# zkHubHQ/distributed-groth16

Hardware: NVIDIA H100
Metric: G1 MSM throughput (BN254 Pippenger, 2^20 pairs per GPU) (higher is better)
Workload: dtype u32x8 Montgomery (256-bit modular integers)

## Files before the change

distributed_groth16_b200/csrc/msm.cu:

```cuda
#include "common.cuh"
#include "glv.cuh"

namespace b200zk {

static const uint32_t KEY_NONE = 0xFFFFFFFFu;

template <class T>
__device__ __forceinline__ T ld16(const T* p) {
    static_assert(sizeof(T) % 16 == 0, "16-byte multiple");
    T r;
    const uint4* s = reinterpret_cast<const uint4*>(p);
    uint4* d = reinterpret_cast<uint4*>(&r);
#pragma unroll
    for (int i = 0; i < (int)(sizeof(T) / 16); ++i) d[i] = s[i];
    return r;
}
template <class T>
__device__ __forceinline__ void st16(T* p, const T& v) {
    static_assert(sizeof(T) % 16 == 0, "16-byte multiple");
    const uint4* s = reinterpret_cast<const uint4*>(&v);
    uint4* d = reinterpret_cast<uint4*>(p);
#pragma unroll
    for (int i = 0; i < (int)(sizeof(T) / 16); ++i) d[i] = s[i];
}
// ... 107 lines not shown
__global__ void __launch_bounds__(SCAN_THREADS) k_scan_sums(uint32_t* sums, uint32_t n) {
    __shared__ uint32_t warp_sums[32];
    __shared__ uint32_t carry_s;
    if (threadIdx.x == 0) carry_s = 0;
    __syncthreads();
    for (uint32_t base = 0; base < n; base += SCAN_THREADS) {
        uint32_t i = base + threadIdx.x;
        uint32_t v = i < n ? sums[i] : 0, total;
        uint32_t ex = block_exclusive_scan(v, &total, warp_sums);
        uint32_t carry = carry_s;
        if (i < n) sums[i] = ex + carry;
        __syncthreads();
        if (threadIdx.x == 0) carry_s = carry + total;
        __syncthreads();
    }
}
__global__ void __launch_bounds__(SCAN_THREADS) k_scan_add(uint32_t* out, const uint32_t* sums, uint32_t n) {
    uint32_t base = blockIdx.x * SCAN_TILE + threadIdx.x * SCAN_ITEMS;
    uint32_t add = sums[blockIdx.x];
#pragma unroll
    for (uint32_t j = 0; j < SCAN_ITEMS; ++j) if (base + j < n) out[base + j] += add;
}

__global__ void k_msm_scatter(const uint32_t* keys, const uint32_t* ranks, const uint32_t* offsets, uint32_t n, size_t t0,
                              size_t total, uint32_t fold, uint32_t* entries) {
    size_t t = (size_t)blockIdx.x * blockDim.x + threadIdx.x;
    if (t >= total) return;
    t += t0;
    uint32_t key = keys[t];
    if (key == KEY_NONE) return;
    uint32_t i = fold ? (uint32_t)t : (uint32_t)(t % n);
    uint32_t g = key & 0x7FFFFFFFu;
    entries[offsets[g] + ranks[t]] = i | (key & 0x80000000u);
}

static const uint32_t TASK_LEN = 128, MAX_TASK_LEN = 1024;
#ifndef B2_ACC_MINBLOCKS
#define B2_ACC_MINBLOCKS 4
#endif
#ifndef B2_ACC_MINBLOCKS_G2
#define B2_ACC_MINBLOCKS_G2 4
#endif

__global__ void k_msm_task_counts(const uint32_t* offsets, uint32_t nbuckets, uint32_t task_len, uint32_t* ntasks) {
    uint32_t g = blockIdx.x * blockDim.x + threadIdx.x;
    if (g > nbuckets) return;
    ntasks[g] = g < nbuckets ? (offsets[g + 1] - offsets[g] + task_len - 1) / task_len : 0;
}

static const uint32_t MERGE_SMALL = 8;
__global__ void k_msm_fill_tasks(const uint32_t* task_off, uint32_t nbuckets, uint32_t* task_bucket, uint32_t* multi_list,
                                 uint32_t list_cap, uint32_t* multi_count) {
    uint32_t g = blockIdx.x * blockDim.x + threadIdx.x;
    if (g >= nbuckets) return;
    uint32_t lo = task_off[g], hi = task_off[g + 1];
    for (uint32_t t = lo; t < hi; ++t) task_bucket[t] = g;
    if (hi - lo > MERGE_SMALL) multi_list[atomicAdd(multi_count, 1u)] = g;
    else if (hi - lo > 1) multi_list[list_cap - 1 - atomicAdd(multi_count + 1, 1u)] = g;
}

__device__ __forceinline__ uint32_t task_length(const uint32_t* offsets, const uint32_t* task_off, uint32_t g, uint32_t t,
                                                uint32_t task_len) {
    uint32_t lo = offsets[g] + (t - task_off[g]) * task_len, end = offsets[g + 1];
    return (lo + task_len < end ? lo + task_len : end) - lo;
}
__global__ void __launch_bounds__(256) k_msm_task_hist(const uint32_t* offsets, const uint32_t* task_off, const uint32_t* task_bucket,
                                uint32_t nbuckets, uint32_t task_len, uint32_t* hist, uint32_t* task_rank) {
    __shared__ uint32_t sh_cnt[MAX_TASK_LEN + 1], sh_base[MAX_TASK_LEN + 1];
    for (uint32_t i = threadIdx.x; i <= task_len; i += blockDim.x) sh_cnt[i] = 0;
    __syncthreads();
    uint32_t t = blockIdx.x * blockDim.x + threadIdx.x;
    bool live = t < task_off[nbuckets];
    uint32_t len = 0, local = 0;
    if (live) {
        len = task_length(offsets, task_off, task_bucket[t], t, task_len);
        local = atomicAdd(sh_cnt + len, 1u);
    }
    __syncthreads();
    for (uint32_t i = threadIdx.x; i <= task_len; i += blockDim.x)
        if (sh_cnt[i]) sh_base[i] = atomicAdd(hist + i, sh_cnt[i]);
    __syncthreads();
    if (live) task_rank[t] = sh_base[len] + local;
}
__global__ void k_msm_task_hist_scan(uint32_t* hist, uint32_t task_len) {
    uint32_t run = 0;
    for (int len = (int)task_len; len >= 0; --len) { uint32_t c = hist[len]; hist[len] = run; run += c; }
}
__global__ void k_msm_task_order(const uint32_t* offsets, const uint32_t* task_off, const uint32_t* task_bucket,
                                 uint32_t nbuckets, uint32_t task_len, const uint32_t* hist, const uint32_t* task_rank,
                                 uint32_t* order) {
    uint32_t t = blockIdx.x * blockDim.x + threadIdx.x;
    if (t >= task_off[nbuckets]) return;
    uint32_t len = task_length(offsets, task_off, task_bucket[t], t, task_len);
    order[hist[len] + task_rank[t]] = t;
}

template <class F, bool RMW>
__global__ void __launch_bounds__(128, sizeof(F) > 32 ? B2_ACC_MINBLOCKS_G2 : B2_ACC_MINBLOCKS) k_msm_accumulate(const affine_t<F>* bases, const uint32_t* entries, const uint32_t* offsets,
                                 const uint32_t* task_off, const uint32_t* task_bucket, const uint32_t* order,
                                 uint32_t nbuckets, uint32_t task_len, uint32_t wave, xyzz_t<F>* buckets, xyzz_t<F>* task_sums) {
    const uint32_t ntask = task_off[nbuckets];
    const uint32_t nblk = (ntask + blockDim.x - 1) / blockDim.x;
    if (blockIdx.x >= nblk) return;
    uint32_t vb = blockIdx.x;
    const uint32_t stride = nblk / wave;
    if (stride > 1) {
        if (vb < wave) vb *= stride;
        else {
            uint32_t j = vb - wave;
            vb = j < wave * (stride - 1) ? (j / (stride - 1)) * stride + j % (stride - 1) + 1 : wave * stride + (j - wave * (stride - 1));
        }
    }
    uint32_t tid = vb * blockDim.x + threadIdx.x;
    if (tid >= ntask) return;
    uint32_t t = order[tid];
    uint32_t g = task_bucket[t];
    uint32_t t0 = task_off[g], nt = task_off[g + 1] - t0;
    uint32_t lo = offsets[g] + (t - t0) * task_len, end = offsets[g + 1];
    uint32_t hi = lo + task_len < end ? lo + task_len : end;
    xyzz_t<F> acc = xyzz_t<F>::identity();
    if (RMW && nt == 1) acc = ld16(buckets + g);
    for (uint32_t k = lo; k < hi; ++k) {
        uint32_t e = entries[k];
        affine_t<F> p = ld16(bases + (e & 0x7FFFFFFFu));
        xyzz_t<F>::madd(acc, p, (e >> 31) != 0);
    }
    if (nt == 1) st16(buckets + g, acc);
    else st16(task_sums + t, acc);
}

template <class F>
__device__ __forceinline__ xyzz_t<F> add_sel(const xyzz_t<F>& a, const xyzz_t<F>& b) {
    if (sizeof(F) == 32) return xyzz_t<F>::add_inl(a, b);
    return xyzz_t<F>::add(a, b);
}

template <class F>
__global__ void __launch_bounds__(128) k_msm_merge_tasks(const uint32_t* multi_list, const uint32_t* multi_count,
                                  const uint32_t* task_off, const xyzz_t<F>* task_sums, uint32_t rmw, xyzz_t<F>* buckets) {
    __shared__ xyzz_t<F> sh[128];
    uint32_t cnt = *multi_count;
    for (uint32_t i = blockIdx.x; i < cnt; i += gridDim.x) {
        uint32_t g = multi_list[i];
        uint32_t lo = task_off[g], hi = task_off[g + 1];
        xyzz_t<F> acc = xyzz_t<F>::identity();
        for (uint32_t t = lo + threadIdx.x; t < hi; t += 128) acc = add_sel<F>(acc, ld16(task_sums + t));
        sh[threadIdx.x] = acc;
        __syncthreads();
        for (int s = 64; s > 0; s >>= 1) {
            if ((int)threadIdx.x < s) {
                xyzz_t<F> a = sh[threadIdx.x], b = sh[threadIdx.x + s];
                sh[threadIdx.x] = add_sel<F>(a, b);
            }
            __syncthreads();
        }
        if (threadIdx.x == 0) st16(buckets + g, rmw ? add_sel<F>(ld16(buckets + g), sh[0]) : sh[0]);
        __syncthreads();
    }
}

template <class F>
__global__ void __launch_bounds__(128) k_msm_merge_small(const uint32_t* multi_list, uint32_t list_cap, const uint32_t* small_count,
                                                         const uint32_t* task_off, const xyzz_t<F>* task_sums, uint32_t rmw, xyzz_t<F>* buckets) {
    uint32_t cnt = *small_count;
    for (uint32_t i = blockIdx.x * blockDim.x + threadIdx.x; i < cnt; i += gridDim.x * blockDim.x) {
        uint32_t g = multi_list[list_cap - 1 - i];
        uint32_t lo = task_off[g], hi = task_off[g + 1];
        xyzz_t<F> acc = ld16(task_sums + lo);
        for (uint32_t t = lo + 1; t < hi; ++t) acc = add_sel<F>(acc, ld16(task_sums + t));
        if (rmw) acc = add_sel<F>(ld16(buckets + g), acc);
        st16(buckets + g, acc);
    }
}

template <class F>
__global__ void __launch_bounds__(128) k_msm_reduce_segments(const xyzz_t<F>* buckets, uint32_t W, uint32_t B, uint32_t seg_len,
                                      xyzz_t<F>* partials) {
    uint32_t nseg = B / seg_len;
    uint32_t t = blockIdx.x * blockDim.x + threadIdx.x;
    if (t >= W * nseg) return;
    uint32_t w = t / nseg, seg = t % nseg;
    uint32_t lo = seg * seg_len;
    const xyzz_t<F>* bw = buckets + (size_t)w * B;
    xyzz_t<F> run = xyzz_t<F>::identity(), acc = xyzz_t<F>::identity();
    constexpr bool INL = sizeof(F) == 32;
    for (uint32_t k = lo + seg_len; k-- > lo;) {
        xyzz_t<F> bk = ld16(bw + k);
        if (INL) { run = xyzz_t<F>::add_inl(run, bk); acc = xyzz_t<F>::add_inl(acc, run); }
        else { run = xyzz_t<F>::add(run, bk); acc = xyzz_t<F>::add(acc, run); }
    }
    if (lo) {
        xyzz_t<F> m = xyzz_t<F>::identity();
        for (int bit = 31 - __clz(lo); bit >= 0; --bit) {
            if (INL) m = xyzz_t<F>::dbl_inl(m); else m = xyzz_t<F>::dbl(m);
            if ((lo >> bit) & 1) { if (INL) m = xyzz_t<F>::add_inl(m, run); else m = xyzz_t<F>::add(m, run); }
        }
        if (INL) acc = xyzz_t<F>::add_inl(acc, m); else acc = xyzz_t<F>::add(acc, m);
    }
    st16(partials + t, acc);
}

template <class F>
__global__ void __launch_bounds__(128) k_msm_reduce_segments_quad(const xyzz_t<F>* buckets, uint32_t W, uint32_t B, uint32_t seg_len,
                                                                  xyzz_t<F>* partials) {
    typedef quad_ops<F, false> Q;
    __shared__ typename Q::xch_t xch[32];
    typename Q::xch_t* x = &xch[threadIdx.x >> 2];
    const uint32_t nseg = B / seg_len;
    const uint32_t t = (blockIdx.x * blockDim.x + threadIdx.x) >> 2;
    if (t >= W * nseg) return;
    const uint32_t w = t / nseg, seg = t % nseg;
    const uint32_t lo = seg * seg_len;
    const xyzz_t<F>* bw = buckets + (size_t)w * B;
    xyzz_t<F> run = xyzz_t<F>::identity(), acc = xyzz_t<F>::identity();
    for (uint32_t k = lo + seg_len; k-- > lo;) {
        run = Q::add(x, run, ld16(bw + k));
        acc = Q::add(x, acc, run);
    }
    if (lo) {
        xyzz_t<F> m = xyzz_t<F>::identity();
        for (int bit = 31 - __clz(lo); bit >= 0; --bit) {
            m = Q::dbl(x, m);
            if ((lo >> bit) & 1) m = Q::add(x, m, run);
        }
        acc = Q::add(x, acc, m);
    }
    if ((threadIdx.x & 3) == 0) st16(partials + t, acc);
}

template <class F, int THREADS>
__global__ void __launch_bounds__(THREADS) k_msm_window_sum(const xyzz_t<F>* partials, uint32_t nseg, xyzz_t<F>* wsum) {
    __shared__ xyzz_t<F> sh[THREADS];
    const xyzz_t<F>* p = partials + (size_t)blockIdx.x * nseg;
    xyzz_t<F> acc = xyzz_t<F>::identity();
    for (uint32_t i = threadIdx.x; i < nseg; i += THREADS) acc = add_sel<F>(acc, ld16(p + i));
    sh[threadIdx.x] = acc;
    __syncthreads();
    for (int s = THREADS / 2; s > 0; s >>= 1) {
        if ((int)threadIdx.x < s) {
            xyzz_t<F> a = sh[threadIdx.x], b = sh[threadIdx.x + s];
            sh[threadIdx.x] = add_sel<F>(a, b);
        }
        __syncthreads();
    }
    if (threadIdx.x == 0) st16(wsum + blockIdx.x, sh[0]);
}

template <class F>
__global__ void __launch_bounds__(32) k_msm_horner(const xyzz_t<F>* wsum, uint32_t nset, uint32_t c, uint32_t first, uint32_t last,
                                                   xyzz_t<F>* state, xyzz_t<F>* out) {
    typedef quad_ops<F, false> Q;
    __shared__ typename Q::xch_t xch;
    if (blockIdx.x != 0 || threadIdx.x >= 4) return;
    xyzz_t<F> total;
    uint32_t k = 0;
    if (first) { total = ld16(wsum); k = 1; }
    else total = ld16(state);
    for (; k < nset; ++k) {
        for (uint32_t j = 0; j < c; ++j) total = Q::dbl(&xch, total);
        total = Q::add(&xch, total, ld16(wsum + k));
    }
    if (threadIdx.x == 0) st16(last ? out : state, total);
}

__device__ __forceinline__ void glv_phi_x(Fq& x) {
    Fq beta;
#pragma unroll
    for (int i = 0; i < 8; ++i) beta.l[i] = GlvParams::beta(i);
    x = Fq::mul(x, beta);
}
__device__ __forceinline__ void glv_phi_x(Fq2& x) {
    Fq beta;
#pragma unroll
    for (int i = 0; i < 8; ++i) beta.l[i] = GlvParams::beta_g2(i);
    x.c0 = Fq::mul(x.c0, beta);
    x.c1 = Fq::mul(x.c1, beta);
}
template <class F>
__global__ void __launch_bounds__(32) k_msm_horner_glv(const xyzz_t<F>* wsum, uint32_t nwin, uint32_t c, uint32_t first, uint32_t last,
                                                       xyzz_t<F>* state, xyzz_t<F>* out) {
    typedef quad_ops<F, false> Q;
    __shared__ typename Q::xch_t xch[2];
    __shared__ xyzz_t<F> h1;
    if (blockIdx.x != 0 || threadIdx.x >= 8) return;
    const uint32_t half = threadIdx.x >> 2;
    xyzz_t<F> total;
    uint32_t k = 0;
    if (first) { total = ld16(wsum + half); k = 1; }
    else total = ld16(state + half);
    for (; k < nwin; ++k) {
        for (uint32_t j = 0; j < c; ++j) total = Q::dbl(&xch[half], total);
        total = Q::add(&xch[half], total, ld16(wsum + 2 * k + half));
    }
    if (!last) {
        if ((threadIdx.x & 3) == 0) st16(state + half, total);
        return;
    }
    if (threadIdx.x == 4) h1 = total;
    __syncwarp(0xFFu);
    if (half == 0) {
        xyzz_t<F> p = h1;
        if (!p.is_inf()) glv_phi_x(p.x);
        total = Q::add(&xch[0], total, p);
        if (threadIdx.x == 0) st16(out, total);
    }
}

template <class F>
__global__ void k_sum_to_affine(const xyzz_t<F>* pts, uint32_t count, affine_t<F>* out, uint64_t* flag) {
    if (threadIdx.x != 0 || blockIdx.x != 0) return;
    xyzz_t<F> acc = xyzz_t<F>::identity();
    for (uint32_t i = 0; i < count; ++i) acc = xyzz_t<F>::add(acc, ld16(pts + i));
    affine_t<F> a = xyzz_t<F>::to_affine(acc);
    st16(out, a);
    *flag = acc.is_inf() ? 1 : 0;
}

template <class F>
__global__ void k_set_identity(xyzz_t<F>* out) {
    if (threadIdx.x == 0 && blockIdx.x == 0) st16(out, xyzz_t<F>::identity());
}

static unsigned choose_window(size_t n) {
    unsigned lg = ceil_log2(n < 2 ? 2 : n);
    int c = (int)lg - 4;
    if (c < 5) c = 5;
    if (c > 20) c = 20;
    const char* env = getenv("B200ZK_MSM_WINDOW");
    if (env) { int v = atoi(env); if (v >= 2 && v <= 24) c = v; }
    return (unsigned)c;
}

static int exclusive_scan(b200zk_ctx* ctx, cudaStream_t st, const uint32_t* in, uint32_t* out, uint32_t* sums, uint32_t n) {
    uint32_t nblk = (n + SCAN_TILE - 1) / SCAN_TILE;
    {
        LaunchScope ls(ctx, st, "msm_scan");
        k_scan_local<<<nblk, SCAN_THREADS, 0, st>>>(in, out, sums, n);
    }
    {
        LaunchScope ls(ctx, st, "msm_scan");
        k_scan_sums<<<1, SCAN_THREADS, 0, st>>>(sums, nblk);
    }
    {
        LaunchScope ls(ctx, st, "msm_scan");
        k_scan_add<<<nblk, SCAN_THREADS, 0, st>>>(out, sums, n);
    }
    return check_launch(ctx, "scan");
}

static cudaEvent_t msm_event(b200zk_ctx* ctx, int ch, size_t idx) {
    std::vector<cudaEvent_t>& v = ctx->msm_events[ch];
    while (v.size() <= idx) {
        cudaEvent_t e = nullptr;
        if (cudaEventCreateWithFlags(&e, cudaEventDisableTiming) != cudaSuccess) return nullptr;
        v.push_back(e);
    }
    return v[idx];
}

struct MsmStreams {
    cudaStream_t seq, acc;
    bool result_on_seq;
    int channel;
};

struct MsmPart {
    const void* bases;
    const void* scalars;
    size_t n;
    cudaEvent_t bases_ready, scalars_ready;
};

template <class F>
static int msm_dev_impl(b200zk_ctx* ctx, const MsmStreams& ms, DevBuf& ws_buf, const MsmPart* parts, unsigned nparts,
                        void* d_out, const char* acc_name, unsigned tab_c = 0, unsigned c_force = 0) {
    const int ch = ms.channel;
    size_t nev = 0;
    auto next_event = [&]() { return msm_event(ctx, ch, nev++); };
    size_t n = 0, n_max = 0;
    for (unsigned p = 0; p < nparts; ++p) { n += parts[p].n; n_max = parts[p].n > n_max ? parts[p].n : n_max; }
    xyzz_t<F>* out = reinterpret_cast<xyzz_t<F>*>(d_out);
    if (n == 0) {
        cudaStream_t rs = ms.result_on_seq ? ms.seq : ms.acc;
        {
            LaunchScope ls(ctx, rs, "msm_small");
            k_set_identity<F><<<1, 32, 0, rs>>>(out);
        }
        return check_launch(ctx, "k_set_identity");
    }
    if (n >= (1ull << 31)) return set_error(ctx, B200ZK_ERR_ARG, "MSM length must be < 2^31");
    const bool fold = tab_c != 0;
    if (fold && nparts != 1) return set_error(ctx, B200ZK_ERR_ARG, "fixed-base tables take one input part");
    const unsigned c = fold ? tab_c : (c_force ? c_force : choose_window(n));
    static const bool glv_env = !(getenv("B200ZK_MSM_GLV") && getenv("B200ZK_MSM_GLV")[0] == '0');
    static const bool glv2_env = !(getenv("B200ZK_MSM_GLV_G2") && getenv("B200ZK_MSM_GLV_G2")[0] == '0');
    const bool glv = !fold && glv_env && (sizeof(F) == 32 || glv2_env);
    const unsigned Wh = (128 + c - 1) / c;
    const unsigned W = glv ? 2 * Wh : (255 + c - 1) / c;
    const unsigned WB = fold ? 1 : W;
    if ((uint64_t)W * n >= (fold ? (1ull << 31) : (1ull << 32)))
        return set_error(ctx, B200ZK_ERR_ARG, "MSM too large for 32-bit bucket offsets / entry indices (W * n)");
    const uint32_t B = 1u << (c - 1);
    const uint32_t nb = WB * B;
    uint32_t seg_len = B < 16 ? B : 16;
    static const bool quad_env = !(getenv("B200ZK_MSM_QUAD_REDUCE") && getenv("B200ZK_MSM_QUAD_REDUCE")[0] == '0');
    const bool quad_reduce = quad_env && (uint64_t)WB * (B / seg_len) <= 8192;
    {
        static const int seg_env = getenv("B200ZK_MSM_SEG") ? atoi(getenv("B200ZK_MSM_SEG")) : 0;
        if (seg_env >= 2 && (seg_env & (seg_env - 1)) == 0 && (uint32_t)seg_env <= B) seg_len = (uint32_t)seg_env;
        else if (quad_reduce) seg_len = B < 8 ? B : 8;
        else if (ctx->msm_seg_hint && ctx->msm_seg_hint <= B) seg_len = ctx->msm_seg_hint;
    }
    const uint32_t nseg = B / seg_len;
    const uint32_t wsplit = fold ? (nseg >= 16 * 256 ? 16 : (nseg >= 1024 ? 4 : 1)) : 1;

    unsigned ngroups = 1;
    if (!fold && nparts == 1) {
        static const int g_env = getenv("B200ZK_MSM_GROUPS") ? atoi(getenv("B200ZK_MSM_GROUPS")) : 0;
        const unsigned nunits = glv ? Wh : W;
        unsigned want = g_env > 0 ? (unsigned)g_env : (n >= (1u << 22) ? 4u : 1u);
        if (want > nunits) want = nunits;
        ngroups = want;
    }
    const unsigned unit_sets = glv ? 2 : 1;
    const unsigned units = (fold ? 1 : (glv ? Wh : W));
    unsigned bounds[17] = {0};
    bool custom_units = false;
    if (!fold && nparts == 1) {
        static const char* gu_env = getenv("B200ZK_MSM_GROUP_UNITS");
        if (gu_env) {
            unsigned k = 0, sum = 0;
            const char* w = gu_env;
            while (*w && k < 16) {
                unsigned v = (unsigned)strtoul(w, const_cast<char**>(&w), 10);
                if (v) { sum += v; bounds[++k] = sum; }
                while (*w == ',' || *w == ' ') ++w;
            }
            if (k >= 1 && sum == units) { custom_units = true; ngroups = k; }
        }
    }
    auto group_first_unit = [&](unsigned g) {
        return custom_units ? bounds[g] : (unsigned)(((uint64_t)units * g) / ngroups);
    };
    const uint32_t rmw = nparts > 1 ? 1u : 0u;

    const bool split_streams = ms.result_on_seq || ngroups > 1 || nparts > 1;
    const cudaStream_t st = split_streams ? ms.seq : ms.acc, ast = ms.acc;
    const bool handshake = split_streams && !ms.result_on_seq;
    if (handshake) {
        cudaEvent_t e = next_event();
        if (!e) return set_error(ctx, B200ZK_ERR_CUDA, "cudaEventCreate failed");
        B2_CUDA_OK(ctx, cudaEventRecord(e, ast));
        B2_CUDA_OK(ctx, cudaStreamWaitEvent(st, e, 0));
    }
    auto finish = [&]() -> int {
        if (handshake) {
            cudaEvent_t e = next_event();
            if (!e) return set_error(ctx, B200ZK_ERR_CUDA, "cudaEventCreate failed");
            B2_CUDA_OK(ctx, cudaEventRecord(e, st));
            B2_CUDA_OK(ctx, cudaStreamWaitEvent(ast, e, 0));
        }
        return B200ZK_OK;
    };

    auto al = [](size_t x) { return (x + 255) & ~(size_t)255; };
    const size_t total_max = (size_t)W * n_max;
    uint32_t task_len = TASK_LEN;
    while (task_len < MAX_TASK_LEN && (uint64_t)task_len * nb < 3 * (uint64_t)total_max &&
           total_max / (2 * task_len) + nb >= (1u << 19))
        task_len *= 2;
    static const bool short_env = !(getenv("B200ZK_MSM_SHORT_TASKS") && getenv("B200ZK_MSM_SHORT_TASKS")[0] == '0');
    if (short_env && n_max <= (1u << 16))
        while (task_len > 16 && total_max / task_len < (1u << 17)) task_len /= 2;
    const size_t max_tasks = total_max / task_len + nb + ngroups;
    size_t o = 0;
    auto carve = [&](size_t bytes) { size_t r = o; o += al(bytes); return r; };
    struct PartWs { size_t keys, ranks, entries, counts, offsets, ntasks, taskoff, taskbucket, multi, hist, rank, order, tasksums; };
    std::vector<PartWs> pw(nparts);
    for (unsigned p = 0; p < nparts; ++p) {
        const size_t total = (size_t)W * parts[p].n;
        pw[p].keys = carve(total * 4); pw[p].ranks = carve(total * 4); pw[p].entries = carve(total * 4);
        pw[p].counts = carve(((size_t)nb + 1) * 4); pw[p].offsets = carve(((size_t)nb + 1) * 4);
        pw[p].ntasks = carve(((size_t)nb + ngroups) * 4); pw[p].taskoff = carve(((size_t)nb + ngroups) * 4);
        pw[p].taskbucket = carve(max_tasks * 4);
        pw[p].multi = carve((total_max / task_len + 4 * ngroups + 4) * 4);
        pw[p].hist = carve((size_t)ngroups * (MAX_TASK_LEN + 1) * 4);
        pw[p].rank = carve(max_tasks * 4); pw[p].order = carve(max_tasks * 4);
        pw[p].tasksums = carve(max_tasks * sizeof(xyzz_t<F>));
    }
    const size_t o_sums = carve(((size_t)nb / SCAN_TILE + 2) * 4);
    const size_t o_buckets = carve((size_t)nb * sizeof(xyzz_t<F>));
    const size_t o_partials = carve((size_t)WB * nseg * sizeof(xyzz_t<F>));
    const size_t o_wsum = carve((size_t)WB * wsplit * sizeof(xyzz_t<F>));
    const size_t o_state = carve(2 * sizeof(xyzz_t<F>));
    B2_CUDA_OK(ctx, ws_buf.reserve(o));
    char* ws = reinterpret_cast<char*>(ws_buf.p);
    uint32_t* sums = reinterpret_cast<uint32_t*>(ws + o_sums);
    xyzz_t<F>* buckets = reinterpret_cast<xyzz_t<F>*>(ws + o_buckets);
    xyzz_t<F>* partials = reinterpret_cast<xyzz_t<F>*>(ws + o_partials);
    xyzz_t<F>* wsum = reinterpret_cast<xyzz_t<F>*>(ws + o_wsum);
    xyzz_t<F>* hstate = reinterpret_cast<xyzz_t<F>*>(ws + o_state);
    B2_CUDA_OK(ctx, cudaMemsetAsync(buckets, 0, (size_t)nb * sizeof(xyzz_t<F>), st));
    cudaEvent_t buckets_clear = nullptr;
    if (rmw) {
        buckets_clear = next_event();
        if (!buckets_clear) return set_error(ctx, B200ZK_ERR_CUDA, "cudaEventCreate failed");
        B2_CUDA_OK(ctx, cudaEventRecord(buckets_clear, st));
        B2_CUDA_OK(ctx, cudaStreamWaitEvent(ast, buckets_clear, 0));
    }

    struct Group {
        uint32_t set0, nsets, b0, nbk;
        size_t task_cap, task_base;
        uint32_t list_cap; size_t list_base;
    };
    std::vector<Group> groups(ngroups);
    {
        size_t tb = 0, lb = 2 * (size_t)ngroups;
        for (unsigned g = 0; g < ngroups; ++g) {
            Group& G = groups[g];
            const unsigned u0 = group_first_unit(g), u1 = group_first_unit(g + 1);
            G.set0 = u0 * unit_sets; G.nsets = (u1 - u0) * unit_sets;
            G.b0 = G.set0 * B; G.nbk = G.nsets * B;
            const size_t gtotal = fold ? total_max : (size_t)G.nsets * n_max;
            G.task_cap = gtotal / task_len + G.nbk + 1;
            G.task_base = tb; tb += G.task_cap;
            G.list_cap = (uint32_t)(gtotal / task_len + 1);
            G.list_base = lb; lb += G.list_cap;
        }
    }
    std::vector<cudaEvent_t> prepped((size_t)nparts * ngroups), accumulated((size_t)nparts * ngroups);
    for (auto& e : prepped) if (!(e = next_event())) return set_error(ctx, B200ZK_ERR_CUDA, "cudaEventCreate failed");
    for (auto& e : accumulated) if (!(e = next_event())) return set_error(ctx, B200ZK_ERR_CUDA, "cudaEventCreate failed");

    bool l2_window = false;
    if (nparts == 1 && ctx->l2_persist_max && ctx->l2_window_max) {
        size_t bytes = n * sizeof(affine_t<F>);
        cudaStreamAttrValue attr;
        memset(&attr, 0, sizeof(attr));
        attr.accessPolicyWindow.base_ptr = const_cast<void*>(parts[0].bases);
        attr.accessPolicyWindow.num_bytes = bytes < ctx->l2_window_max ? bytes : ctx->l2_window_max;
        double ratio = (double)ctx->l2_persist_max / (double)attr.accessPolicyWindow.num_bytes;
        attr.accessPolicyWindow.hitRatio = ratio > 1.0 ? 1.0f : (float)ratio;
        attr.accessPolicyWindow.hitProp = cudaAccessPropertyPersisting;
        attr.accessPolicyWindow.missProp = cudaAccessPropertyStreaming;
        l2_window = cudaStreamSetAttribute(ast, cudaStreamAttributeAccessPolicyWindow, &attr) == cudaSuccess;
        cudaGetLastError();
    }

    for (unsigned p = 0; p < nparts; ++p) {
        const MsmPart& P = parts[p];
        const size_t np = P.n, total = (size_t)W * np;
        uint32_t* keys = reinterpret_cast<uint32_t*>(ws + pw[p].keys);
        uint32_t* ranks = reinterpret_cast<uint32_t*>(ws + pw[p].ranks);
        uint32_t* entries = reinterpret_cast<uint32_t*>(ws + pw[p].entries);
        uint32_t* counts = reinterpret_cast<uint32_t*>(ws + pw[p].counts);
        uint32_t* offsets = reinterpret_cast<uint32_t*>(ws + pw[p].offsets);
        uint32_t* ntasks_all = reinterpret_cast<uint32_t*>(ws + pw[p].ntasks);
        uint32_t* task_off_all = reinterpret_cast<uint32_t*>(ws + pw[p].taskoff);
        uint32_t* task_bucket_all = reinterpret_cast<uint32_t*>(ws + pw[p].taskbucket);
        uint32_t* multi_all = reinterpret_cast<uint32_t*>(ws + pw[p].multi);
        uint32_t* hist_all = reinterpret_cast<uint32_t*>(ws + pw[p].hist);
        uint32_t* task_rank_all = reinterpret_cast<uint32_t*>(ws + pw[p].rank);
        uint32_t* order_all = reinterpret_cast<uint32_t*>(ws + pw[p].order);
        xyzz_t<F>* task_sums_all = reinterpret_cast<xyzz_t<F>*>(ws + pw[p].tasksums);
        if (np == 0) {
            for (unsigned g = 0; g < ngroups; ++g) {
                B2_CUDA_OK(ctx, cudaEventRecord(prepped[(size_t)p * ngroups + g], st));
                B2_CUDA_OK(ctx, cudaEventRecord(accumulated[(size_t)p * ngroups + g], ast));
            }
            continue;
        }
        if (P.scalars_ready) B2_CUDA_OK(ctx, cudaStreamWaitEvent(st, P.scalars_ready, 0));
        B2_CUDA_OK(ctx, cudaMemsetAsync(counts, 0, ((size_t)nb + 1) * 4, st));
        {
            LaunchScope ls(ctx, st, "msm_digits");
            if (glv) k_msm_digits_glv<<<(unsigned)((np + 255) / 256), 256, 0, st>>>(reinterpret_cast<const Fr*>(P.scalars), (uint32_t)np, c,
                                                                                   Wh, keys, ranks, counts);
            else k_msm_digits<<<(unsigned)((np + 255) / 256), 256, 0, st>>>(reinterpret_cast<const Fr*>(P.scalars), (uint32_t)np, c, W,
                                                                              fold ? 1u : 0u, keys, ranks, counts);
        }
        B2_TRY(check_launch(ctx, "k_msm_digits"));
        B2_TRY(exclusive_scan(ctx, st, counts, offsets, sums, nb + 1));
        B2_CUDA_OK(ctx, cudaMemsetAsync(multi_all, 0, (size_t)ngroups * 8, st));
        B2_CUDA_OK(ctx, cudaMemsetAsync(hist_all, 0, (size_t)ngroups * (MAX_TASK_LEN + 1) * 4, st));

        for (unsigned g = 0; g < ngroups; ++g) {
            const Group& G = groups[g];
            uint32_t* ntasks = ntasks_all + G.b0 + g;
            uint32_t* task_off = task_off_all + G.b0 + g;
            uint32_t* task_bucket = task_bucket_all + G.task_base;
            uint32_t* task_rank = task_rank_all + G.task_base;
            uint32_t* order = order_all + G.task_base;
            uint32_t* hist = hist_all + (size_t)g * (MAX_TASK_LEN + 1);
            {
                LaunchScope ls(ctx, st, "msm_tasks");
                k_msm_task_counts<<<(G.nbk + 1 + 255) / 256, 256, 0, st>>>(offsets + G.b0, G.nbk, task_len, ntasks);
            }
            B2_TRY(check_launch(ctx, "k_msm_task_counts"));
            B2_TRY(exclusive_scan(ctx, st, ntasks, task_off, sums, G.nbk + 1));
            {
                LaunchScope ls(ctx, st, "msm_tasks");
                k_msm_fill_tasks<<<(G.nbk + 255) / 256, 256, 0, st>>>(task_off, G.nbk, task_bucket, multi_all + G.list_base, G.list_cap,
                                                                      multi_all + 2 * g);
            }
            B2_TRY(check_launch(ctx, "k_msm_fill_tasks"));
            {
                LaunchScope ls(ctx, st, "msm_tasks");
                k_msm_task_hist<<<(unsigned)((G.task_cap + 255) / 256), 256, 0, st>>>(offsets + G.b0, task_off, task_bucket, G.nbk, task_len, hist, task_rank);
            }
            {
                LaunchScope ls(ctx, st, "msm_tasks");
                k_msm_task_hist_scan<<<1, 1, 0, st>>>(hist, task_len);
            }
            {
                LaunchScope ls(ctx, st, "msm_tasks");
                k_msm_task_order<<<(unsigned)((G.task_cap + 255) / 256), 256, 0, st>>>(offsets + G.b0, task_off, task_bucket, G.nbk, task_len, hist, task_rank, order);
            }
            B2_TRY(check_launch(ctx, "k_msm_task_order"));
            {
                const size_t t0 = fold ? 0 : (size_t)G.set0 * np, cnt = fold ? total : (size_t)G.nsets * np;
                LaunchScope ls(ctx, st, "msm_scatter");
                k_msm_scatter<<<(unsigned)((cnt + 255) / 256), 256, 0, st>>>(keys, ranks, offsets, (uint32_t)np, t0, cnt, fold ? 1u : 0u, entries);
            }
            B2_TRY(check_launch(ctx, "k_msm_scatter"));
            B2_CUDA_OK(ctx, cudaEventRecord(prepped[(size_t)p * ngroups + g], st));
        }

        if (P.bases_ready) B2_CUDA_OK(ctx, cudaStreamWaitEvent(ast, P.bases_ready, 0));
        for (unsigned g = 0; g < ngroups; ++g) {
            const Group& G = groups[g];
            B2_CUDA_OK(ctx, cudaStreamWaitEvent(ast, prepped[(size_t)p * ngroups + g], 0));
            {
                LaunchScope ls(ctx, ast, acc_name);
                const unsigned grid = (unsigned)((G.task_cap + 127) / 128);
                const uint32_t wave = (uint32_t)ctx->sm_count * (sizeof(F) > 32 ? B2_ACC_MINBLOCKS_G2 : B2_ACC_MINBLOCKS);
                const affine_t<F>* bp = reinterpret_cast<const affine_t<F>*>(P.bases);
                if (rmw) k_msm_accumulate<F, true><<<grid, 128, 0, ast>>>(bp, entries, offsets + G.b0, task_off_all + G.b0 + g, task_bucket_all + G.task_base,
                                                                       order_all + G.task_base, G.nbk, task_len, wave, buckets + G.b0, task_sums_all + G.task_base);
                else k_msm_accumulate<F, false><<<grid, 128, 0, ast>>>(bp, entries, offsets + G.b0, task_off_all + G.b0 + g, task_bucket_all + G.task_base,
                                                                        order_all + G.task_base, G.nbk, task_len, wave, buckets + G.b0, task_sums_all + G.task_base);
            }
            B2_TRY(check_launch(ctx, "k_msm_accumulate"));
            if (rmw) {
                {
                    LaunchScope ls(ctx, ast, "msm_merge");
                    k_msm_merge_tasks<F><<<2 * ctx->sm_count, 128, 0, ast>>>(multi_all + G.list_base, multi_all + 2 * g, task_off_all + G.b0 + g,
                                                                            task_sums_all + G.task_base, rmw, buckets + G.b0);
                }
                {
                    LaunchScope ls(ctx, ast, "msm_merge");
                    k_msm_merge_small<F><<<4 * ctx->sm_count, 128, 0, ast>>>(multi_all + G.list_base, G.list_cap, multi_all + 2 * g + 1,
                                                                            task_off_all + G.b0 + g, task_sums_all + G.task_base, rmw, buckets + G.b0);
                }
                B2_TRY(check_launch(ctx, "k_msm_merge_tasks"));
            }
            B2_CUDA_OK(ctx, cudaEventRecord(accumulated[(size_t)p * ngroups + g], ast));
        }
    }
    if (l2_window) {
        cudaStreamAttrValue attr;
        memset(&attr, 0, sizeof(attr));
        attr.accessPolicyWindow.num_bytes = 0;
        cudaStreamSetAttribute(ast, cudaStreamAttributeAccessPolicyWindow, &attr);
        cudaGetLastError();
    }

    for (unsigned g = 0; g < ngroups; ++g) {
        const Group& G = groups[g];
        for (unsigned p = 0; p < nparts; ++p) B2_CUDA_OK(ctx, cudaStreamWaitEvent(st, accumulated[(size_t)p * ngroups + g], 0));
        if (!rmw) {
            uint32_t* multi_all = reinterpret_cast<uint32_t*>(ws + pw[0].multi);
            uint32_t* task_off = reinterpret_cast<uint32_t*>(ws + pw[0].taskoff) + G.b0 + g;
            xyzz_t<F>* task_sums = reinterpret_cast<xyzz_t<F>*>(ws + pw[0].tasksums) + G.task_base;
            {
                LaunchScope ls(ctx, st, "msm_merge");
                k_msm_merge_tasks<F><<<2 * ctx->sm_count, 128, 0, st>>>(multi_all + G.list_base, multi_all + 2 * g, task_off, task_sums, 0u, buckets + G.b0);
            }
            {
                LaunchScope ls(ctx, st, "msm_merge");
                k_msm_merge_small<F><<<4 * ctx->sm_count, 128, 0, st>>>(multi_all + G.list_base, G.list_cap, multi_all + 2 * g + 1, task_off, task_sums,
                                                                       0u, buckets + G.b0);
            }
            B2_TRY(check_launch(ctx, "k_msm_merge_tasks"));
        }
        {
            LaunchScope ls(ctx, st, "msm_reduce");
            if (quad_reduce)
                k_msm_reduce_segments_quad<F><<<(G.nsets * nseg * 4 + 127) / 128, 128, 0, st>>>(buckets + G.b0, G.nsets, B, seg_len,
                                                                                               partials + (size_t)G.set0 * nseg);
            else
                k_msm_reduce_segments<F><<<(G.nsets * nseg + 127) / 128, 128, 0, st>>>(buckets + G.b0, G.nsets, B, seg_len,
                                                                                      partials + (size_t)G.set0 * nseg);
        }
        B2_TRY(check_launch(ctx, "k_msm_reduce_segments"));
        {
            LaunchScope ls(ctx, st, "msm_window_sum");
            constexpr int T = sizeof(F) > 32 ? 128 : 256;
            k_msm_window_sum<F, T><<<G.nsets * wsplit, T, 0, st>>>(partials + (size_t)G.set0 * nseg, nseg / wsplit, wsum + (size_t)G.set0 * wsplit);
        }
        B2_TRY(check_launch(ctx, "k_msm_window_sum"));
        {
            LaunchScope ls(ctx, st, "msm_combine");
            const uint32_t first = g == 0, last = g + 1 == ngroups;
            if (glv) k_msm_horner_glv<F><<<1, 32, 0, st>>>(wsum + G.set0, G.nsets / 2, c, first, last, hstate, out);
            else k_msm_horner<F><<<1, 32, 0, st>>>(wsum + (size_t)G.set0 * wsplit, G.nsets * wsplit, fold ? 0u : c, first, last, hstate, out);
        }
        B2_TRY(check_launch(ctx, "k_msm_horner"));
    }
    return finish();
}

template <class F>
static int msm_dev_impl(b200zk_ctx* ctx, const MsmStreams& ms, DevBuf& ws_buf, const void* d_bases, const void* d_scalars, size_t n,
                        void* d_out, const char* acc_name, cudaEvent_t bases_ready, cudaEvent_t scalars_ready = nullptr,
                        unsigned tab_c = 0, unsigned c_force = 0) {
    const MsmPart part{d_bases, d_scalars, n, bases_ready, scalars_ready};
    return msm_dev_impl<F>(ctx, ms, ws_buf, &part, 1, d_out, acc_name, tab_c, c_force);
}

static MsmStreams slot_streams(b200zk_ctx* ctx, Slot& sl, int aux) {
    const int ch = 2 * (int)(&sl - ctx->slots) + (aux ? 1 : 0);
    return MsmStreams{ctx->msm_side[ch], aux ? sl.aux_stream : sl.stream, false, ch};
}

int msm_g1_dev(b200zk_ctx* ctx, Slot& sl, const void* d_bases, const void* d_scalars, size_t n, void* d_out,
               cudaEvent_t bases_ready, int aux) {
    return msm_dev_impl<Fq>(ctx, slot_streams(ctx, sl, aux), aux ? sl.ws_msm_aux : sl.ws_msm, d_bases, d_scalars, n, d_out,
                            "msm_accumulate_g1", bases_ready);
}
int msm_g2_dev(b200zk_ctx* ctx, Slot& sl, const void* d_bases, const void* d_scalars, size_t n, void* d_out,
               cudaEvent_t bases_ready, int aux) {
    return msm_dev_impl<Fq2>(ctx, slot_streams(ctx, sl, aux), aux ? sl.ws_msm_aux : sl.ws_msm, d_bases, d_scalars, n, d_out,
                             "msm_accumulate_g2", bases_ready);
}

unsigned msm_table_windows(unsigned c) { return (255 + c - 1) / c; }
unsigned msm_table_auto_window(size_t n) {
    int L = (int)ceil_log2(n < 2 ? 2 : n);
    L = L < 10 ? 10 : (L > 20 ? 20 : L);
    const int cand[4] = {L, L - 1, L + 1, L - 2};
    for (int c : cand) {
        if (c < 10 || c > 20) continue;
        int top = 254 - ((int)msm_table_windows((unsigned)c) - 1) * c;
        if (top >= 6) return (unsigned)c;
    }
    return (unsigned)L;
}

template <class F>
__global__ void __launch_bounds__(128) k_msm_table_build(const affine_t<F>* bases, uint32_t n, uint32_t c, uint32_t W,
                                                         affine_t<F>* table) {
    uint32_t i = blockIdx.x * blockDim.x + threadIdx.x;
    if (i >= n) return;
    affine_t<F> p = ld16(bases + i);
    st16(table + i, p);
    for (uint32_t w = 1; w < W; ++w) {
        if (!p.is_inf()) {
            xyzz_t<F> acc = xyzz_t<F>::from_affine(p);
            for (uint32_t k = 0; k < c; ++k) acc = xyzz_t<F>::dbl(acc);
            p = xyzz_t<F>::to_affine(acc);
        }
        st16(table + (size_t)w * n + i, p);
    }
}

template <class F>
static int table_build_impl(b200zk_ctx* ctx, cudaStream_t st, const void* d_bases, size_t n, unsigned c, void* d_table) {
    if (c < 2 || c > 24) return set_error(ctx, B200ZK_ERR_ARG, "table window must be in [2, 24]");
    if (n == 0) return B200ZK_OK;
    const unsigned W = msm_table_windows(c);
    if ((uint64_t)W * n >= (1ull << 31)) return set_error(ctx, B200ZK_ERR_ARG, "table too large (W * n >= 2^31)");
    {
        LaunchScope ls(ctx, st, "msm_table_build");
        k_msm_table_build<F><<<(unsigned)((n + 127) / 128), 128, 0, st>>>(reinterpret_cast<const affine_t<F>*>(d_bases), (uint32_t)n,
                                                                      c, W, reinterpret_cast<affine_t<F>*>(d_table));
    }
    return check_launch(ctx, "k_msm_table_build");
}
int msm_table_build_dev(b200zk_ctx* ctx, Slot& sl, int g2, const void* d_bases, size_t n, unsigned c, void* d_table) {
    return g2 ? table_build_impl<Fq2>(ctx, sl.stream, d_bases, n, c, d_table)
              : table_build_impl<Fq>(ctx, sl.stream, d_bases, n, c, d_table);
}
int msm_table_dev(b200zk_ctx* ctx, Slot& sl, int g2, const void* d_table, const void* d_scalars, size_t n, unsigned c,
                  void* d_out, int aux) {
    if (c < 2 || c > 24) return set_error(ctx, B200ZK_ERR_ARG, "table window must be in [2, 24]");
    const MsmStreams st = slot_streams(ctx, sl, aux);
    DevBuf& ws = aux ? sl.ws_msm_aux : sl.ws_msm;
    return g2 ? msm_dev_impl<Fq2>(ctx, st, ws, d_table, d_scalars, n, d_out, "msm_accumulate_g2", nullptr, nullptr, c)
              : msm_dev_impl<Fq>(ctx, st, ws, d_table, d_scalars, n, d_out, "msm_accumulate_g1", nullptr, nullptr, c);
}
// ... 206 lines not shown
```

Before: 223.4.

## Replace per-segment offset multiply with hierarchical tree reduction of bucket segments

The segment reduction no longer computes the lo*run correction by double-and-add per thread. It emits both the running sum and the weighted sum for each segment, and a new multi-level shared-memory tree kernel combines segments, applying the offset weights with a few doublings per level. This removes a long serial double-and-add chain per segment and the separate window-sum kernel, at the cost of extra launches per level and larger shared-memory use. The single-threaded task-length histogram scan is also replaced by a block-wide parallel scan.

```diff
diff --git a/distributed_groth16_b200/csrc/msm.cu b/distributed_groth16_b200/csrc/msm.cu
--- a/distributed_groth16_b200/csrc/msm.cu
+++ b/distributed_groth16_b200/csrc/msm.cu
@@ -213,9 +213,24 @@
     __syncthreads();
     if (live) task_rank[t] = sh_base[len] + local;
 }
-__global__ void k_msm_task_hist_scan(uint32_t* hist, uint32_t task_len) {
-    uint32_t run = 0;
-    for (int len = (int)task_len; len >= 0; --len) { uint32_t c = hist[len]; hist[len] = run; run += c; }
+__global__ void __launch_bounds__(SCAN_THREADS) k_msm_task_hist_scan(uint32_t* hist, uint32_t task_len) {
+    constexpr uint32_t ITEMS = (MAX_TASK_LEN + SCAN_THREADS) / SCAN_THREADS;
+    __shared__ uint32_t warp_sums[32];
+    uint32_t v[ITEMS], t = 0;
+#pragma unroll
+    for (uint32_t j = 0; j < ITEMS; ++j) {
+        const uint32_t r = threadIdx.x * ITEMS + j;
+        v[j] = r <= task_len ? hist[task_len - r] : 0;
+        t += v[j];
+    }
+    uint32_t total;
+    uint32_t ex = block_exclusive_scan(t, &total, warp_sums);
+#pragma unroll
+    for (uint32_t j = 0; j < ITEMS; ++j) {
+        const uint32_t r = threadIdx.x * ITEMS + j;
+        if (r <= task_len) hist[task_len - r] = ex;
+        ex += v[j];
+    }
 }
 __global__ void k_msm_task_order(const uint32_t* offsets, const uint32_t* task_off, const uint32_t* task_bucket,
                                  uint32_t nbuckets, uint32_t task_len, const uint32_t* hist, const uint32_t* task_rank,
@@ -306,7 +321,7 @@
 
 template <class F>
 __global__ void __launch_bounds__(128) k_msm_reduce_segments(const xyzz_t<F>* buckets, uint32_t W, uint32_t B, uint32_t seg_len,
-                                      xyzz_t<F>* partials) {
+                                      xyzz_t<F>* ys, xyzz_t<F>* gs) {
     uint32_t nseg = B / seg_len;
     uint32_t t = blockIdx.x * blockDim.x + threadIdx.x;
     if (t >= W * nseg) return;
@@ -320,20 +335,13 @@
         if (INL) { run = xyzz_t<F>::add_inl(run, bk); acc = xyzz_t<F>::add_inl(acc, run); }
         else { run = xyzz_t<F>::add(run, bk); acc = xyzz_t<F>::add(acc, run); }
     }
-    if (lo) {
-        xyzz_t<F> m = xyzz_t<F>::identity();
-        for (int bit = 31 - __clz(lo); bit >= 0; --bit) {
-            if (INL) m = xyzz_t<F>::dbl_inl(m); else m = xyzz_t<F>::dbl(m);
-            if ((lo >> bit) & 1) { if (INL) m = xyzz_t<F>::add_inl(m, run); else m = xyzz_t<F>::add(m, run); }
-        }
-        if (INL) acc = xyzz_t<F>::add_inl(acc, m); else acc = xyzz_t<F>::add(acc, m);
-    }
-    st16(partials + t, acc);
+    st16(ys + t, run);
+    st16(gs + t, acc);
 }
 
 template <class F>
 __global__ void __launch_bounds__(128) k_msm_reduce_segments_quad(const xyzz_t<F>* buckets, uint32_t W, uint32_t B, uint32_t seg_len,
-                                                                  xyzz_t<F>* partials) {
+                                                                  xyzz_t<F>* ys, xyzz_t<F>* gs) {
     typedef quad_ops<F, false> Q;
     __shared__ typename Q::xch_t xch[32];
     typename Q::xch_t* x = &xch[threadIdx.x >> 2];
@@ -356,26 +364,54 @@
         }
         acc = Q::add(x, acc, m);
     }
-    if ((threadIdx.x & 3) == 0) st16(partials + t, acc);
-}
-
-template <class F, int THREADS>
-__global__ void __launch_bounds__(THREADS) k_msm_window_sum(const xyzz_t<F>* partials, uint32_t nseg, xyzz_t<F>* wsum) {
-    __shared__ xyzz_t<F> sh[THREADS];
-    const xyzz_t<F>* p = partials + (size_t)blockIdx.x * nseg;
+    if ((threadIdx.x & 3) == 0) { st16(ys + t, xyzz_t<F>::identity()); st16(gs + t, acc); }
+}
+
+template <class F>
+__global__ void k_msm_reduce_level(const xyzz_t<F>* yin, const xyzz_t<F>* gin, uint32_t lgT, uint32_t lgf, xyzz_t<F>* yout,
+                                   xyzz_t<F>* hout) {
+    typedef quad_ops<F, false> Q;
+    extern __shared__ uint4 smem_raw[];
+    xyzz_t<F>* sY = reinterpret_cast<xyzz_t<F>*>(smem_raw);
+    const uint32_t T = 1u << lgT, tid = threadIdx.x;
+    xyzz_t<F>* sG = sY + T;
+    xyzz_t<F>* sP = sG + T;
+    __shared__ typename Q::xch_t xch;
+    const size_t base = (size_t)blockIdx.x * T;
+    if (tid < T) { sY[tid] = ld16(yin + base + tid); sG[tid] = ld16(gin + base + tid); }
+    __syncthreads();
+    for (uint32_t l = 0; l < lgT; ++l) {
+        const uint32_t nn = T >> (l + 1), jobs = nn * (l + 2);
+        xyzz_t<F> r;
+        uint32_t j = 0, kind = 0;
+        if (tid < jobs) {
+            j = tid % nn; kind = tid / nn;
+            const xyzz_t<F>* src = kind == 0 ? sY : kind == 1 ? sG : sP + T - (T >> (kind - 2));
+            r = add_sel<F>(src[2 * j], src[2 * j + 1]);
+            if (kind == 0) sP[T - (T >> l) + j] = src[2 * j + 1];
+        }
+        __syncthreads();
+        if (tid < jobs) {
+            xyzz_t<F>* dst = kind == 0 ? sY : kind == 1 ? sG : sP + T - (T >> (kind - 2));
+            dst[j] = r;
+        }
+        __syncthreads();
+    }
+    if (tid >= 4) return;
     xyzz_t<F> acc = xyzz_t<F>::identity();
-    for (uint32_t i = threadIdx.x; i < nseg; i += THREADS) acc = add_sel<F>(acc, ld16(p + i));
-    sh[threadIdx.x] = acc;
-    __syncthreads();
-    for (int s = THREADS / 2; s > 0; s >>= 1) {
-        if ((int)threadIdx.x < s) {
-            xyzz_t<F> a = sh[threadIdx.x], b = sh[threadIdx.x + s];
-            sh[threadIdx.x] = add_sel<F>(a, b);
-        }
-        __syncthreads();
-    }
-    if (threadIdx.x == 0) st16(wsum + blockIdx.x, sh[0]);
-}
+    for (int jj = (int)lgT - 1; jj >= 0; --jj) {
+        acc = Q::dbl(&xch, acc);
+        acc = Q::add(&xch, acc, sP[T - (T >> jj)]);
+    }
+    for (uint32_t k = 0; k < lgf; ++k) acc = Q::dbl(&xch, acc);
+    acc = Q::add(&xch, sG[0], acc);
+    if (tid == 0) {
+        st16(hout + blockIdx.x, acc);
+        if (yout) st16(yout + blockIdx.x, sY[0]);
+    }
+}
+template <class F> constexpr uint32_t reduce_level_lgtmax() { return sizeof(F) > 32 ? 7 : 8; }
+template <class F> constexpr size_t reduce_level_smem(uint32_t lgT) { return (size_t)(3u << lgT) * sizeof(xyzz_t<F>); }
 
 template <class F>
 __global__ void __launch_bounds__(32) k_msm_horner(const xyzz_t<F>* wsum, uint32_t nset, uint32_t c, uint32_t first, uint32_t last,
@@ -543,7 +579,8 @@
         else if (ctx->msm_seg_hint && ctx->msm_seg_hint <= B) seg_len = ctx->msm_seg_hint;
     }
     const uint32_t nseg = B / seg_len;
-    const uint32_t wsplit = fold ? (nseg >= 16 * 256 ? 16 : (nseg >= 1024 ? 4 : 1)) : 1;
+    constexpr uint32_t LGT_MAX = reduce_level_lgtmax<F>();
+    const uint32_t nlev2 = nseg > (1u << LGT_MAX) ? nseg >> LGT_MAX : 1;
 
     unsigned ngroups = 1;
     if (!fold && nparts == 1) {
@@ -621,14 +658,16 @@
     }
     const size_t o_sums = carve(((size_t)nb / SCAN_TILE + 2) * 4);
     const size_t o_buckets = carve((size_t)nb * sizeof(xyzz_t<F>));
-    const size_t o_partials = carve((size_t)WB * nseg * sizeof(xyzz_t<F>));
-    const size_t o_wsum = carve((size_t)WB * wsplit * sizeof(xyzz_t<F>));
+    const size_t o_lev1 = carve(2 * (size_t)WB * nseg * sizeof(xyzz_t<F>));
+    const size_t o_lev2 = carve(2 * (size_t)WB * nlev2 * sizeof(xyzz_t<F>));
+    const size_t o_wsum = carve((size_t)WB * sizeof(xyzz_t<F>));
     const size_t o_state = carve(2 * sizeof(xyzz_t<F>));
     B2_CUDA_OK(ctx, ws_buf.reserve(o));
     char* ws = reinterpret_cast<char*>(ws_buf.p);
     uint32_t* sums = reinterpret_cast<uint32_t*>(ws + o_sums);
     xyzz_t<F>* buckets = reinterpret_cast<xyzz_t<F>*>(ws + o_buckets);
-    xyzz_t<F>* partials = reinterpret_cast<xyzz_t<F>*>(ws + o_partials);
+    xyzz_t<F>* lev1 = reinterpret_cast<xyzz_t<F>*>(ws + o_lev1);
+    xyzz_t<F>* lev2 = reinterpret_cast<xyzz_t<F>*>(ws + o_lev2);
     xyzz_t<F>* wsum = reinterpret_cast<xyzz_t<F>*>(ws + o_wsum);
     xyzz_t<F>* hstate = reinterpret_cast<xyzz_t<F>*>(ws + o_state);
     B2_CUDA_OK(ctx, cudaMemsetAsync(buckets, 0, (size_t)nb * sizeof(xyzz_t<F>), st));
@@ -742,7 +781,7 @@
             }
             {
                 LaunchScope ls(ctx, st, "msm_tasks");
-                k_msm_task_hist_scan<<<1, 1, 0, st>>>(hist, task_len);
+                k_msm_task_hist_scan<<<1, SCAN_THREADS, 0, st>>>(hist, task_len);
             }
             {
                 LaunchScope ls(ctx, st, "msm_tasks");
@@ -816,26 +855,44 @@
             B2_TRY(check_launch(ctx, "k_msm_merge_tasks"));
         }
         {
+            xyzz_t<F>* ys = lev1 + (size_t)G.set0 * nseg;
+            xyzz_t<F>* gs = lev1 + (size_t)WB * nseg + (size_t)G.set0 * nseg;
             LaunchScope ls(ctx, st, "msm_reduce");
             if (quad_reduce)
-                k_msm_reduce_segments_quad<F><<<(G.nsets * nseg * 4 + 127) / 128, 128, 0, st>>>(buckets + G.b0, G.nsets, B, seg_len,
-                                                                                               partials + (size_t)G.set0 * nseg);
+                k_msm_reduce_segments_quad<F><<<(G.nsets * nseg * 4 + 127) / 128, 128, 0, st>>>(buckets + G.b0, G.nsets, B, seg_len, ys, gs);
             else
-                k_msm_reduce_segments<F><<<(G.nsets * nseg + 127) / 128, 128, 0, st>>>(buckets + G.b0, G.nsets, B, seg_len,
-                                                                                      partials + (size_t)G.set0 * nseg);
+                k_msm_reduce_segments<F><<<(G.nsets * nseg + 127) / 128, 128, 0, st>>>(buckets + G.b0, G.nsets, B, seg_len, ys, gs);
         }
         B2_TRY(check_launch(ctx, "k_msm_reduce_segments"));
         {
-            LaunchScope ls(ctx, st, "msm_window_sum");
-            constexpr int T = sizeof(F) > 32 ? 128 : 256;
-            k_msm_window_sum<F, T><<<G.nsets * wsplit, T, 0, st>>>(partials + (size_t)G.set0 * nseg, nseg / wsplit, wsum + (size_t)G.set0 * wsplit);
-        }
-        B2_TRY(check_launch(ctx, "k_msm_window_sum"));
+            B2_CUDA_OK(ctx, cudaFuncSetAttribute(k_msm_reduce_level<F>, cudaFuncAttributeMaxDynamicSharedMemorySize,
+                                                 (int)reduce_level_smem<F>(LGT_MAX)));
+            uint32_t n = nseg, lgf = ceil_log2(seg_len);
+            bool from1 = true;
+            for (;;) {
+                uint32_t lgT = ceil_log2(n);
+                if (lgT > LGT_MAX) lgT = LGT_MAX;
+                const uint32_t nb = n >> lgT, T = 1u << lgT;
+                xyzz_t<F>* in = from1 ? lev1 : lev2;
+                const size_t icap = from1 ? nseg : nlev2, ocap = from1 ? nlev2 : nseg;
+                xyzz_t<F>* outb = from1 ? lev2 : lev1;
+                {
+                    LaunchScope ls(ctx, st, "msm_reduce");
+                    k_msm_reduce_level<F><<<G.nsets * nb, T < 32 ? 32 : T, reduce_level_smem<F>(lgT), st>>>(
+                        in + (size_t)G.set0 * n, in + (size_t)WB * icap + (size_t)G.set0 * n, lgT, lgf,
+                        nb == 1 ? nullptr : outb + (size_t)G.set0 * nb,
+                        nb == 1 ? wsum + G.set0 : outb + (size_t)WB * ocap + (size_t)G.set0 * nb);
+                }
+                B2_TRY(check_launch(ctx, "k_msm_reduce_level"));
+                if (nb == 1) break;
+                n = nb; lgf += lgT; from1 = !from1;
+            }
+        }
         {
             LaunchScope ls(ctx, st, "msm_combine");
             const uint32_t first = g == 0, last = g + 1 == ngroups;
             if (glv) k_msm_horner_glv<F><<<1, 32, 0, st>>>(wsum + G.set0, G.nsets / 2, c, first, last, hstate, out);
-            else k_msm_horner<F><<<1, 32, 0, st>>>(wsum + (size_t)G.set0 * wsplit, G.nsets * wsplit, fold ? 0u : c, first, last, hstate, out);
+            else k_msm_horner<F><<<1, 32, 0, st>>>(wsum + G.set0, G.nsets, fold ? 0u : c, first, last, hstate, out);
         }
         B2_TRY(check_launch(ctx, "k_msm_horner"));
     }
```

Measured after the change: 227.8, median of 6. About the same (+1.9%).

## Replace segment bucket reduction with hierarchical pairwise level reduction

Applied to the files above, without the earlier changes.

Adds a multi-level bucket-sum reduction. A first kernel computes per-segment running and weighted sums and scales the running sum by doublings. Pairwise kernels then combine adjacent segments up a tree until one value per window remains. This replaces the per-segment scalar multiply by segment offset and the separate window-sum kernel, cutting group operations in the reduce phase. The cost is several extra small kernel launches and extra workspace for the level buffers.

```diff
diff --git a/distributed_groth16_b200/csrc/msm.cu b/distributed_groth16_b200/csrc/msm.cu
--- a/distributed_groth16_b200/csrc/msm.cu
+++ b/distributed_groth16_b200/csrc/msm.cu
@@ -359,6 +359,57 @@
     if ((threadIdx.x & 3) == 0) st16(partials + t, acc);
 }
 
+static const uint32_t MSM_LEVEL1_LEN = 16;
+
+template <class F>
+__global__ void __launch_bounds__(128, sizeof(F) > 32 ? 1 : 4) k_msm_reduce_level1(const xyzz_t<F>* buckets, uint32_t nsets, uint32_t B,
+                                                                                uint32_t lg, xyzz_t<F>* Xo, xyzz_t<F>* Yo) {
+    const uint32_t L = 1u << lg, nseg = (B + L - 1) >> lg;
+    const uint32_t t = blockIdx.x * blockDim.x + threadIdx.x;
+    if (t >= nsets * nseg) return;
+    const uint32_t set = t / nseg, seg = t % nseg;
+    const uint32_t lo = seg << lg, hi = lo + L < B ? lo + L : B;
+    const xyzz_t<F>* b = buckets + (size_t)set * B;
+    constexpr bool INL = sizeof(F) == 32;
+    xyzz_t<F> run = xyzz_t<F>::identity(), acc = xyzz_t<F>::identity();
+    for (uint32_t k = hi; k-- > lo;) {
+        xyzz_t<F> bk = ld16(b + k);
+        if (INL) { run = xyzz_t<F>::add_inl(run, bk); acc = xyzz_t<F>::add_inl(acc, run); }
+        else { run = xyzz_t<F>::add(run, bk); acc = xyzz_t<F>::add(acc, run); }
+    }
+    st16(Yo + t, acc);
+    if (nseg > 1) {
+        for (uint32_t i = 0; i < lg; ++i) { if (INL) run = xyzz_t<F>::dbl_inl(run); else run = xyzz_t<F>::dbl(run); }
+        st16(Xo + t, run);
+    }
+}
+
+template <class F>
+__global__ void __launch_bounds__(128) k_msm_reduce_pairs(const xyzz_t<F>* X, const xyzz_t<F>* Y, uint32_t nsets, uint32_t m,
+                                                          xyzz_t<F>* Xo, xyzz_t<F>* Yo) {
+    typedef quad_ops<F, false> Q;
+    __shared__ typename Q::xch_t xch[32];
+    typename Q::xch_t* q = &xch[threadIdx.x >> 2];
+    const uint32_t nseg = (m + 1) >> 1;
+    const uint32_t t = blockIdx.x * 16 + ((threadIdx.x & 63) >> 2);
+    const bool x_role = threadIdx.x >= 64;
+    if (t >= nsets * nseg || (x_role && nseg == 1)) return;
+    const uint32_t set = t / nseg, j = 2 * (t % nseg);
+    const bool pair = j + 1 < m;
+    const xyzz_t<F>* x = X + (size_t)set * m;
+    xyzz_t<F> r;
+    if (x_role) {
+        r = ld16(x + j);
+        if (pair) r = Q::add(q, r, ld16(x + j + 1));
+        r = Q::dbl(q, r);
+    } else {
+        const xyzz_t<F>* y = Y + (size_t)set * m;
+        r = ld16(y + j);
+        if (pair) { r = Q::add(q, r, ld16(y + j + 1)); r = Q::add(q, r, ld16(x + j + 1)); }
+    }
+    if ((threadIdx.x & 3) == 0) st16((x_role ? Xo : Yo) + t, r);
+}
+
 template <class F, int THREADS>
 __global__ void __launch_bounds__(THREADS) k_msm_window_sum(const xyzz_t<F>* partials, uint32_t nseg, xyzz_t<F>* wsum) {
     __shared__ xyzz_t<F> sh[THREADS];
@@ -536,14 +587,23 @@
     uint32_t seg_len = B < 16 ? B : 16;
     static const bool quad_env = !(getenv("B200ZK_MSM_QUAD_REDUCE") && getenv("B200ZK_MSM_QUAD_REDUCE")[0] == '0');
     const bool quad_reduce = quad_env && (uint64_t)WB * (B / seg_len) <= 8192;
+    static const bool segments_env = getenv("B200ZK_MSM_REDUCE") && !strcmp(getenv("B200ZK_MSM_REDUCE"), "segments");
+    const bool levels = !quad_reduce && !segments_env;
     {
         static const int seg_env = getenv("B200ZK_MSM_SEG") ? atoi(getenv("B200ZK_MSM_SEG")) : 0;
         if (seg_env >= 2 && (seg_env & (seg_env - 1)) == 0 && (uint32_t)seg_env <= B) seg_len = (uint32_t)seg_env;
         else if (quad_reduce) seg_len = B < 8 ? B : 8;
+        else if (levels) seg_len = B < MSM_LEVEL1_LEN ? B : MSM_LEVEL1_LEN;
         else if (ctx->msm_seg_hint && ctx->msm_seg_hint <= B) seg_len = ctx->msm_seg_hint;
     }
     const uint32_t nseg = B / seg_len;
-    const uint32_t wsplit = fold ? (nseg >= 16 * 256 ? 16 : (nseg >= 1024 ? 4 : 1)) : 1;
+    const uint32_t wsplit = fold && !levels ? (nseg >= 16 * 256 ? 16 : (nseg >= 1024 ? 4 : 1)) : 1;
+    std::vector<uint32_t> lv_m;
+    std::vector<size_t> lv_off;
+    size_t lv_elems = 0;
+    if (levels) {
+        for (uint32_t m = nseg; m > 1; m = (m + 1) / 2) { lv_m.push_back(m); lv_off.push_back(lv_elems); lv_elems += m; }
+    }
 
     unsigned ngroups = 1;
     if (!fold && nparts == 1) {
@@ -621,7 +681,7 @@
     }
     const size_t o_sums = carve(((size_t)nb / SCAN_TILE + 2) * 4);
     const size_t o_buckets = carve((size_t)nb * sizeof(xyzz_t<F>));
-    const size_t o_partials = carve((size_t)WB * nseg * sizeof(xyzz_t<F>));
+    const size_t o_partials = carve((levels ? 2 * lv_elems : (size_t)nseg) * WB * sizeof(xyzz_t<F>));
     const size_t o_wsum = carve((size_t)WB * wsplit * sizeof(xyzz_t<F>));
     const size_t o_state = carve(2 * sizeof(xyzz_t<F>));
     B2_CUDA_OK(ctx, ws_buf.reserve(o));
@@ -797,6 +857,15 @@
         cudaGetLastError();
     }
 
+    auto horner = [&](uint32_t s0, uint32_t ns, bool first, bool last) -> int {
+        {
+            LaunchScope ls(ctx, st, "msm_combine");
+            if (glv) k_msm_horner_glv<F><<<1, 32, 0, st>>>(wsum + s0, ns / 2, c, first, last, hstate, out);
+            else k_msm_horner<F><<<1, 32, 0, st>>>(wsum + (size_t)s0 * wsplit, ns * wsplit, fold ? 0u : c, first, last, hstate, out);
+        }
+        return check_launch(ctx, "k_msm_horner");
+    };
+
     for (unsigned g = 0; g < ngroups; ++g) {
         const Group& G = groups[g];
         for (unsigned p = 0; p < nparts; ++p) B2_CUDA_OK(ctx, cudaStreamWaitEvent(st, accumulated[(size_t)p * ngroups + g], 0));
@@ -815,6 +884,31 @@
             }
             B2_TRY(check_launch(ctx, "k_msm_merge_tasks"));
         }
+        if (levels) {
+            xyzz_t<F>* xs = partials;
+            xyzz_t<F>* ys = partials + WB * lv_elems;
+            auto level_out = [&](xyzz_t<F>* base, size_t i, uint32_t s0) { return base + (WB * lv_off[i] + (size_t)s0 * lv_m[i]); };
+            xyzz_t<F>* fin = fold ? out : wsum + G.set0;
+            {
+                LaunchScope ls(ctx, st, "msm_reduce");
+                const bool one = lv_m.empty();
+                k_msm_reduce_level1<F><<<(G.nsets * nseg + 127) / 128, 128, 0, st>>>(buckets + G.b0, G.nsets, B, 31 - __builtin_clz(seg_len),
+                                                                                     one ? nullptr : level_out(xs, 0, G.set0),
+                                                                                     one ? fin : level_out(ys, 0, G.set0));
+            }
+            B2_TRY(check_launch(ctx, "k_msm_reduce_level1"));
+            for (size_t i = 0; i < lv_m.size(); ++i) {
+                const bool last = i + 1 == lv_m.size();
+                const uint32_t ns = (lv_m[i] + 1) / 2;
+                LaunchScope ls(ctx, st, "msm_reduce_upper");
+                k_msm_reduce_pairs<F><<<(G.nsets * ns + 15) / 16, 128, 0, st>>>(level_out(xs, i, G.set0), level_out(ys, i, G.set0), G.nsets, lv_m[i],
+                                                                               last ? nullptr : level_out(xs, i + 1, G.set0),
+                                                                               last ? fin : level_out(ys, i + 1, G.set0));
+            }
+            B2_TRY(check_launch(ctx, "k_msm_reduce_pairs"));
+            if (!fold) B2_TRY(horner(G.set0, G.nsets, g == 0, g + 1 == ngroups));
+            continue;
+        }
         {
             LaunchScope ls(ctx, st, "msm_reduce");
             if (quad_reduce)
@@ -831,13 +925,7 @@
             k_msm_window_sum<F, T><<<G.nsets * wsplit, T, 0, st>>>(partials + (size_t)G.set0 * nseg, nseg / wsplit, wsum + (size_t)G.set0 * wsplit);
         }
         B2_TRY(check_launch(ctx, "k_msm_window_sum"));
-        {
-            LaunchScope ls(ctx, st, "msm_combine");
-            const uint32_t first = g == 0, last = g + 1 == ngroups;
-            if (glv) k_msm_horner_glv<F><<<1, 32, 0, st>>>(wsum + G.set0, G.nsets / 2, c, first, last, hstate, out);
-            else k_msm_horner<F><<<1, 32, 0, st>>>(wsum + (size_t)G.set0 * wsplit, G.nsets * wsplit, fold ? 0u : c, first, last, hstate, out);
-        }
-        B2_TRY(check_launch(ctx, "k_msm_horner"));
+        B2_TRY(horner(G.set0, G.nsets, g == 0, g + 1 == ngroups));
     }
     return finish();
 }
```

New measurement: 221.9 before, 227.5 after, median of 6. 1.03x the previous value.
